# yusupov1alik/MPI-Jordan-crazy-acceleration

Measured on AMD Instinct MI355X. Metric: GFLOP/s + wall-clock, N=32768 dense Gauss-Jordan at 1/2/4/8 MI355X, higher is better.
Workload: dtype fp64

## Files before the change

### csrc/include/gj/device.hpp

```cpp
#pragma once

#include <cmath>
#include <limits>
#include <memory>
#include <string>

#include "gj/common.hpp"
#include "gj/layout.hpp"
#include "gj/pivot.hpp"

namespace gj {

enum class GenKind : int { AbsDiff = 0, Hilbert = 1, Identity = 2, Random = 3, Zero = 4, RandomShifted = 5 };

struct GenSpec {
  GenKind kind = GenKind::AbsDiff;
  uint64_t seed = 0;
};

enum class GemmOp : int { Acc = 0, Store = 1 };
enum class ALayout : int { RowMajor = 0, KMajor = 1 };

struct GemmExtra {
  static constexpr int kMaxZeroRows = 8;
  int64_t zc0 = 0, zc1 = 0;
  int nzr = 0;
  int64_t zr[kMaxZeroRows] = {};
  int64_t zh = 0;
  bool latency = false;
  bool lat_wide = false;
  bool lat_reg = false;
  void* tneg = nullptr;
  int64_t ldtneg = 0;
  int64_t tneg_cols = 0;
  int64_t skip_c0 = 0, skip_c1 = 0;
  const int32_t* owner_phys = nullptr;
  int64_t owner_p = 1, owner_k = 0;
  bool dense = false;
  int glds_build = 0;
  int glds_tile = 0;
  int c_nt = -1;
  const void* c_in = nullptr;
  int64_t ldc_in = 0;
  static constexpr int kRselWords = 8;
  uint64_t rsel[kRselWords] = {};
  int64_t rsel_m = 0;
  int64_t rsel_count() const {
    int64_t c = 0;
    for (int w = 0; w < kRselWords; ++w) c += __builtin_popcountll(rsel[w]);
    return c;
  }
  int64_t rsel_row(int64_t i) const {
    int64_t bl = i / rsel_m;
    const int64_t off = i - bl * rsel_m;
    for (int w = 0; w < kRselWords; ++w) {
      uint64_t x = rsel[w];
      const int c = __builtin_popcountll(x);
      if (bl < c) {
        for (; bl > 0; --bl) x &= x - 1;
        return (64 * w + __builtin_ctzll(x)) * rsel_m + off;
      }
// ... 215 lines not shown
```

### csrc/kernels/gemm.hip

```cpp
#include <hip/hip_runtime.h>

#include <stdexcept>

#include <cstdint>
#include <cstdlib>
#include <string>
#include <type_traits>
#include <utility>

#include "kernels.hpp"

namespace gj {
namespace kern {

constexpr int PADL = 16;
constexpr int kRecords = 0x7ffffff0;
constexpr int kOOB = 0x7ffffff8;

template <int BM_, int BN_, int BK_, int WM_, int WN_, int OCC_, int PF_ = 1>
struct Cfg {
  static constexpr int BM = BM_, BN = BN_, BK = BK_, WM = WM_, WN = WN_, OCC = OCC_;
  static constexpr int PF = PF_;
  static constexpr int NT = 64 * WM * WN;
  static constexpr int TM = BM / WM, TN = BN / WN;
// ... 89 lines not shown
struct GemmArgs {
  int64_t M, N, K;
  const void* A;
  int64_t lda;
  const void* B;
  int64_t ldb;
  void* C;
  int64_t ldc;
  int tiles_m, tiles_n;
  int64_t zc0, zc1;
  int64_t zr[GemmExtra::kMaxZeroRows];
  int64_t zh;
  int64_t n_real, blk_m, p, k;
  double* partial;
  int nparts;
  bool latency;
  bool lat_wide;
  bool lat_reg;
  bool c_overlap;
  int group;
  void* tneg;
  int64_t ldt, tncols;
  const int32_t* pred;
  int64_t pred_p, pred_k;
  bool dense;
  int build;
  int tile;
  uint64_t rsel[GemmExtra::kRselWords];
  int64_t rsel_m;
  int64_t skc0, skc1;
  const void* cin;
  int64_t ldcin;
  int c_nt;
};

__device__ __forceinline__ int64_t rsel_map(const GemmArgs& g, int64_t r) {
  int64_t bl = r / g.rsel_m;
  const int64_t off = r - bl * g.rsel_m;
#pragma unroll
  for (int w = 0; w < GemmExtra::kRselWords; ++w) {
    uint64_t x = g.rsel[w];
    const int c = __popcll(x);
    if (bl < c) {
      for (; bl > 0; --bl) x &= x - 1;
      return (64 * w + __ffsll((unsigned long long)x) - 1) * g.rsel_m + off;
    }
    bl -= c;
  }
  return 0;
}

__device__ __forceinline__ bool gemm_skipped(const GemmArgs& g) {
  if (g.pred == nullptr) return false;
  const int64_t gg = *g.pred;
  return gg < 0 || gg % g.pred_p != g.pred_k;
}

__device__ __forceinline__ int xcd_remap(int bid, int nwg) {
  const int q = nwg / 8, r = nwg % 8, x = bid % 8;
  return (x < r ? x * (q + 1) : r * (q + 1) + (x - r) * q) + bid / 8;
}

template <typename T, int AL, int MODE, typename CF>
__device__ __forceinline__ void gemm_tile(const GemmArgs& g, const int tile) {
  using MF = Mfma<T>;
  using acc_t = typename MF::acc_t;
// ... 307 lines not shown
  const int rlane = wm * TM + MF::rl(lane);
  const int clane = wn * TN + (lane & 15);
  const int Mt = (int)((g.M - m0L) < BM ? (g.M - m0L) : BM);
  const int Nt = (int)((g.N - n0) < BN ? (g.N - n0) : BN);
  const int64_t zlo = g.zc0 - n0, zhi = g.zc1 - n0;
  const int z0 = (int)(zlo < 0 ? 0 : (zlo > BN ? BN : zlo)), z1 = (int)(zhi < 0 ? 0 : (zhi > BN ? BN : zhi));
  int zr0[GemmExtra::kMaxZeroRows], zr1[GemmExtra::kMaxZeroRows];
#pragma unroll
  for (int z = 0; z < GemmExtra::kMaxZeroRows; ++z) {
    const int64_t lo = g.zr[z] - m0, hi = g.zr[z] + g.zh - m0;
    zr0[z] = (int)(lo < 0 ? 0 : (lo > BM ? BM : lo));
    zr1[z] = (int)(hi < 0 ? 0 : (hi > BM ? BM : hi));
  }
  __amdgpu_buffer_rsrc_t rc = rsrc(C + m0 * g.ldc + n0);
  const int cvoff = (rlane * ldc + clane) * ES;

  acc_t acc[MI][NJ];
  const int ldi = g.cin ? (int)g.ldcin : ldc;
  const __amdgpu_buffer_rsrc_t rci = g.cin ? rsrc(static_cast<const double*>(g.cin) + m0 * g.ldcin + n0) : rc;
  const int civoff = (rlane * ldi + clane) * ES;
  bool uni = Mt == BM && Nt == BN && g.cin == nullptr && g.rsel_m == 0;
  bool zin = MODE != MODE_ACC;
  if (MODE == MODE_ACC) {
    uni = uni && (z1 <= z0 || (z0 == 0 && z1 == BN));
    zin = z1 > z0;
#pragma unroll
    for (int z = 0; z < GemmExtra::kMaxZeroRows; ++z) {
      const int h = zr1[z] - zr0[z];
      uni = uni && (h <= 0 || h == BM);
      zin = zin || h > 0;
    }
  }
  if (g.tneg) uni = uni && (n0 >= g.tncols || n0 + BN <= g.tncols);
  auto load_c_masked = [&]() {
#pragma unroll
    for (int i = 0; i < MI; ++i)
#pragma unroll
      for (int q = 0; q < 4; ++q) {
        const int r = rlane + i * 16 + MF::rq(q);
        const int soff = (i * 16 + MF::rq(q)) * ldi * ES;
        bool zrow = false;
#pragma unroll
        for (int z = 0; z < GemmExtra::kMaxZeroRows; ++z) zrow |= (r >= zr0[z] && r < zr1[z]);
#pragma unroll
        for (int j = 0; j < NJ; ++j) {
          const int c = clane + j * 16;
          if (MODE == MODE_ACC) {
            const bool ok = r < Mt && c < Nt && !zrow && !(c >= z0 && c < z1);
            acc[i][j][q] = bload_c(rci, ok ? civoff + j * 16 * ES : kOOB, soff, g.c_nt & 1);
          } else {
            acc[i][j][q] = 0.0;
          }
        }
      }
  };
  auto load_c_uniform = [&](auto nt_c) {
#pragma unroll
    for (int i = 0; i < MI; ++i)
#pragma unroll
      for (int q = 0; q < 4; ++q) {
        const int soff = (i * 16 + MF::rq(q)) * ldc * ES;
#pragma unroll
        for (int j = 0; j < NJ; ++j) acc[i][j][q] = bload_c(rc, cvoff + j * 16 * ES, soff, decltype(nt_c)::value);
      }
  };
  auto load_c = [&]() {
    if (!uni) {
      load_c_masked();
    } else if (zin) {
#pragma unroll
      for (int i = 0; i < MI; ++i)
#pragma unroll
        for (int j = 0; j < NJ; ++j)
#pragma unroll
          for (int q = 0; q < 4; ++q) acc[i][j][q] = 0.0;
    } else if (g.c_nt & 1) {
      load_c_uniform(std::true_type{});
    } else {
      load_c_uniform(std::false_type{});
    }
  };
  if (!(MODE == MODE_ACC && g.c_overlap)) {
    load_c();
#pragma unroll
    for (int i = 0; i < MI; ++i)
#pragma unroll
      for (int j = 0; j < NJ; ++j)
#pragma unroll
        for (int q = 0; q < 4; ++q) asm volatile("" ::"v"(acc[i][j][q]));
  }

  const int acol = 2 * lane;
  const bool a_ok = (m0L + acol) < g.M;
  const int brow = BN == 128 ? wid : 2 * wid + (lane >> 5);
  const int bpos = BN == 128 ? 2 * lane : 2 * (lane & 31);
  const int bcol = bpos ^ ((brow & 1) * 16);
  const bool b_ok = (n0 + bcol) < g.N;
  auto brow_h = [&](int h) { return BN == 128 ? brow + 4 * h : brow + 8 * h; };
  auto blds_h = [&](int h) { return BN == 128 ? (wid + 4 * h) * BN : 2 * (wid + 4 * h) * BN; };
  __amdgpu_buffer_rsrc_t ra = rsrc(A + m0);
  __amdgpu_buffer_rsrc_t rb = rsrc(B + n0);
  const int Kd = (int)g.K;
  auto issue = [&](int kt) {
    double* st = lds + (kt % NS) * STAGE;
    const int k0 = kt * BK;
#pragma unroll
    for (int h = 0; h < BK / 4; ++h) {
      const int kr = wid + 4 * h;
      const bool ok = a_ok && (k0 + kr) < Kd;
      dma16(ra, st + kr * LDA, ok ? ((k0 + kr) * lda + acol) * ES : kOOB);
    }
#pragma unroll
    for (int h = 0; h < BPW; ++h) {
      const int br = brow_h(h);
      const bool okb = b_ok && (k0 + br) < Kd;
      dma16(rb, st + SA + blds_h(h), okb ? ((k0 + br) * ldb + bcol) * ES : kOOB);
    }
  };
  auto compute = [&](int kt) {
    const double* sa = lds + (kt % NS) * STAGE;
    const double* sb = sa + SA;
#pragma unroll
    for (int kk = 0; kk < BK; kk += 4) {
      double a[MI], b[NJ];
      const int kr = kk + (lane >> 4);
      const int sw = (kr & 1) * 16;
#pragma unroll
      for (int i = 0; i < MI; ++i) a[i] = sa[kr * LDA + wm * TM + i * 16 + (lane & 15)];
#pragma unroll
      for (int j = 0; j < NJ; ++j) b[j] = sb[kr * BN + ((wn * TN + j * 16 + (lane & 15)) ^ sw)];
#pragma unroll
      for (int i = 0; i < MI; ++i)
#pragma unroll
        for (int j = 0; j < NJ; ++j) acc[i][j] = MF::op(a[i], b[j], acc[i][j]);
    }
  };

  const int nk = (int)((g.K + BK - 1) / BK);
  const int pro = nk < NS - 1 ? nk : NS - 1;
  if constexpr (PEEL == 0) {
    for (int kt = 0; kt < pro; ++kt) issue(kt);
    if (MODE == MODE_ACC && g.c_overlap) {
      load_c();
      asm volatile("s_waitcnt vmcnt(0)" ::: "memory");
    } else {
      wait_pieces<PIECES>(pro - 1);
    }
    __builtin_amdgcn_s_barrier();
    for (int kt = 0; kt < nk; ++kt) {
      if (kt + NS - 1 < nk) issue(kt + NS - 1);
      compute(kt);
      const int last = (kt + NS - 1 < nk ? kt + NS - 1 : nk - 1);
      wait_pieces<PIECES>(last - (kt + 1) > 0 ? last - (kt + 1) : 0);
      asm volatile("s_waitcnt lgkmcnt(0)" ::: "memory");
      __builtin_amdgcn_s_barrier();
    }
  } else {
    const int nfull = Kd / BK;
    int va[BK / 4], vb[BPW];
#pragma unroll
    for (int h = 0; h < BK / 4; ++h) va[h] = a_ok ? ((wid + 4 * h) * lda + acol) * ES : kOOB;
#pragma unroll
    for (int h = 0; h < BPW; ++h) vb[h] = b_ok ? (brow_h(h) * ldb + bcol) * ES : kOOB;
    const int sa_step = __builtin_amdgcn_readfirstlane(BK * lda * ES);
    const int sb_step = __builtin_amdgcn_readfirstlane(BK * ldb * ES);
    for (int kt = 0; kt < pro; ++kt) issue(kt);
    if (MODE == MODE_ACC && g.c_overlap) {
      load_c();
      asm volatile("s_waitcnt vmcnt(0)" ::: "memory");
    } else {
      wait_pieces<PIECES>(pro - 1);
// ... 271 lines not shown
}
void set_glds_peel(int on) { g_glds_peel = on ? 1 : 0; }
static int g_glds_build = -1;
static int glds_build_forced() {
  if (g_glds_build < 0) {
    const char* e = getenv("GJ_GLDS_BUILD");
    const std::string v = e ? e : "";
    g_glds_build = v.empty() ? 0 : v == "2.5" ? 25 : v == "3.3" ? 33 : v == "2.3" ? 23 : v == "4.3" ? 43
                                                  : v == "16.2.3" ? 1623 : v == "3.2" ? 32 : -2;
    if (g_glds_build == -2) throw std::invalid_argument("GJ_GLDS_BUILD: 2.3 | 2.5 | 3.3 | 4.3 | 16.2.3 | 3.2");
  }
  return g_glds_build;
}
void set_glds_build(int b) {
  if (b != 0 && b != 23 && b != 25 && b != 33 && b != 43 && b != 1623 && b != 32)
    throw std::invalid_argument("glds build: 0 | 23 | 25 | 32 | 33 | 43 | 1623");
  g_glds_build = b;
}

static int g_glds_tile = -1;
static int glds_tile(const GemmArgs& a) {
  if (g_glds_tile < 0) {
    const char* e = getenv("GJ_GLDS_TILE");
    const int v = e ? std::atoi(e) : 0;
    if (v != 0 && v != 64 && v != 128) throw std::invalid_argument("GJ_GLDS_TILE: 64 | 128");
    g_glds_tile = v;
  }
  return g_glds_tile ? g_glds_tile : a.tile == 64 ? 64 : 128;
}
void set_glds_tile(int bn) {
  if (bn != 0 && bn != 64 && bn != 128) throw std::invalid_argument("glds tile: 0 (per launch) | 64 | 128");
  g_glds_tile = bn;
}

static int glds_cnt(int per_launch) {
  static const int forced = [] {
    const char* e = getenv("GJ_GLDS_CNT");
    return e ? (std::atoi(e) & 3) : -1;
  }();
  return forced >= 0 ? forced : per_launch > 0 ? (per_launch & 3) : 0;
}

static int glds_group() {
  static const int g = [] {
    const char* e = getenv("GJ_GLDS_GROUP");
    const int v = e ? std::atoi(e) : 4;
    return v > 0 ? v : 4;
  }();
  return g;
}

template <int MODE>
static void launch_glds(const GemmArgs& a0, hipStream_t s) {
  GemmArgs a = a0;
  const int forced0 = glds_build_forced();
  const int build0 = forced0 ? forced0 : a.build ? a.build : a.dense ? 25 : 23;
  if (glds_tile(a) == 128 && glds_peel() && build0 != 25) {
    a.tiles_m = (int)((a.M + glds::BM - 1) / glds::BM);
    a.tiles_n = (int)((a.N + 127) / 128);
    const int64_t nwg = (int64_t)a.tiles_m * a.tiles_n;
    if (nwg <= 0) return;
    a.group = glds_group();
    a.c_nt = glds_cnt(a.c_nt);
    g_last_gemm_kernel = build0 == 33 ? "glds64:t128:b33:peel" : build0 == 32 ? "glds64:t128:b32:peel" : "glds64:t128:b23:peel";
    if (build0 == 33)
      hipLaunchKernelGGL((gemm_glds_f64<MODE, 3, 3, 8, 1, 128>), dim3((unsigned)nwg), dim3(glds::NT), 0, s, a);
// ... 419 lines not shown
    case 9: return launch_cfg<T, AL, MODE, CfgBigPf>(a, s);
    default: return launch_cfg<T, AL, MODE, CfgBig>(a, s);
  }
}

static void fill_extra(GemmArgs& a, const GemmExtra* ex) {
  constexpr int64_t kNone = -(int64_t(1) << 62);
  a.zc0 = ex ? ex->zc0 : 0;
  a.zc1 = ex ? ex->zc1 : 0;
  a.zh = ex ? ex->zh : 0;
  for (int z = 0; z < GemmExtra::kMaxZeroRows; ++z) a.zr[z] = (ex && z < ex->nzr) ? ex->zr[z] : kNone;
  a.latency = ex ? ex->latency : false;
  a.lat_wide = ex ? ex->lat_wide : false;
  a.lat_reg = ex ? ex->lat_reg : false;
  a.c_overlap = glds_covl();
  a.tneg = ex ? ex->tneg : nullptr;
  a.ldt = ex ? ex->ldtneg : 0;
  a.tncols = (ex && ex->tneg_cols > 0) ? ex->tneg_cols : (int64_t(1) << 62);
  a.pred = ex ? ex->owner_phys : nullptr;
  a.pred_p = ex ? ex->owner_p : 1;
  a.pred_k = ex ? ex->owner_k : 0;
  a.dense = ex ? ex->dense : false;
  a.build = ex ? ex->glds_build : 0;
  a.tile = ex ? ex->glds_tile : 0;
  a.c_nt = ex ? ex->c_nt : -1;
  a.rsel_m = ex ? ex->rsel_m : 0;
  a.cin = ex ? ex->c_in : nullptr;
  a.skc0 = ex ? ex->skip_c0 : 0;
  a.skc1 = ex ? ex->skip_c1 : 0;
  if (a.skc1 > a.skc0 && (a.skc0 % 128 != 0 || a.skc1 % 128 != 0))
    throw Error(Status::BadArgs, "gemm: skip columns must be multiples of 128");
  a.ldcin = ex ? ex->ldc_in : 0;
  for (int w = 0; w < GemmExtra::kRselWords; ++w) a.rsel[w] = ex ? ex->rsel[w] : 0;
}

void gemm(DType dt, int op, int a_kmajor, int64_t M, int64_t N, int64_t K, const void* A,
          int64_t lda, const void* B, int64_t ldb, void* C, int64_t ldc, hipStream_t s,
          const GemmExtra* ex) {
  if (M <= 0 || N <= 0) return;
  GemmArgs a{};
  a.M = M; a.N = N; a.K = K; a.A = A; a.lda = lda; a.B = B; a.ldb = ldb; a.C = C; a.ldc = ldc;
  fill_extra(a, ex);
  if (a.tneg && a.ldt * 128 * (dt == DType::F64 ? 8 : 4) >= kRecords)
    throw Error(Status::BadArgs, "gemm: -C^T leading dimension too large for 32-bit buffer offsets");
  const int mode = op == 0 ? MODE_ACC : MODE_STORE;
#define GJ_DISPATCH(T)                                                        \
  if (a_kmajor) {                                                             \
    if (mode == MODE_ACC) launch<T, 1, MODE_ACC>(a, s);                       \
    else launch<T, 1, MODE_STORE>(a, s);                                      \
  } else {                                                                    \
    if (mode == MODE_ACC) launch<T, 0, MODE_ACC>(a, s);                       \
    else launch<T, 0, MODE_STORE>(a, s);                                      \
  }
  if (dt == DType::F64) {
    GJ_DISPATCH(double)
  } else {
    GJ_DISPATCH(float)
  }
#undef GJ_DISPATCH
}

void gemm_batch(DType dt, const GemmDesc* d, int n, hipStream_t s) {
  using CF = CfgSmall;
  static const bool lat_batch = !getenv("GJ_LAT_BATCH") || std::atoi(getenv("GJ_LAT_BATCH")) != 0;
  bool lat = lat_batch && dt == DType::F64 && n > 0;
  for (int e = 0; e < n && lat; ++e) {
// ... 74 lines not shown
```

### csrc/kernels/kernels.hpp

```cpp
#pragma once

#include <hip/hip_runtime.h>

#include "gj/common.hpp"
#include "gj/device.hpp"
#include "gj/layout.hpp"
#include "gj/pivot.hpp"

namespace gj {
namespace kern {

void gemm(DType dt, int op , int a_kmajor, int64_t M, int64_t N, int64_t K,
          const void* A, int64_t lda, const void* B, int64_t ldb, void* C, int64_t ldc,
          hipStream_t s, const GemmExtra* ex = nullptr);
void gemm_batch(DType dt, const GemmDesc* d, int n, hipStream_t s);
const char* last_gemm_kernel();
int residual_nparts(int64_t N);
int gemm_variant_id(const char* name);
void set_gemm_variant(int v);
void set_glds_peel(int on);
void set_glds_covl(int on);
void set_lat_glds(int on);
void set_lat_kernel(int mode);
void set_glds_build(int b);
void set_glds_tile(int bn);
void set_block_inverse_variant(int v);
int block_inverse_variant();
int block_inverse_variant_id(const char* name);
const char* block_inverse_kernel_name(DType dt, int64_t m, int variant);
void residual_partial(DType dt, int64_t M, int64_t N, int64_t K, const void* A, int64_t lda,
                      const void* B, int64_t ldb, int64_t n_real, int64_t blk_m, int64_t p,
                      int64_t k, double* partial, hipStream_t s);

void candidate_maxabs(DType dt, const void* Lt, int64_t ldl, double* scores, int32_t* valid,
                      const int32_t* used, const Layout& L, double thresh, hipStream_t s);
void gather_candidate(DType dt, void* sel, const void* Lt, int64_t ldl, const PivotRec* rec, const Layout& L,
                      hipStream_t s);
void commit_candidate(DType dt, void* inv_t, const void* inv1, const int32_t* valid1, const double* score1, double growth, PivotRec* rec,
                      const Layout& L, hipStream_t s);

void block_inverse(DType dt, const void* Lt, int64_t ldl, void* inv_t, double* scores,
                   int32_t* valid, const int32_t* used, const Layout& L, double thresh, int64_t nlive,
                   hipStream_t s, void* scratch, int* iscratch, int variant = -1);
bool block_inverse_mfma(DType dt, const void* Lt, int64_t ldl, void* inv_t, double* scores,
                        int32_t* valid, const int32_t* used, const Layout& L, double thresh, int64_t nlive,
                        hipStream_t s, const PivotSelectArgs* sel = nullptr);
bool block_inverse_select(DType dt, const void* Lt, int64_t ldl, void* inv_t, double* scores,
                          int32_t* valid, const int32_t* used, const Layout& L, double thresh, int64_t nlive,
                          hipStream_t s, const PivotSelectArgs& sel, int variant = -1, void* scratch = nullptr);
void set_block_inverse_probe(int32_t* piv_out);
int32_t* block_inverse_probe();
bool block_inverse_big(DType dt, const void* Lt, int64_t ldl, void* inv_t, double* scores, int32_t* valid,
                       const int32_t* used, const Layout& L, double thresh, int64_t nlive, hipStream_t s, void* scratch);
size_t block_inverse_big_scratch_bytes(DType dt, const Layout& L);
void block_inverse_huge(DType dt, const void* Lt, int64_t ldl, void* inv_t, double* scores, int32_t* valid,
                        const int32_t* used, const Layout& L, double thresh, int64_t nlive, hipStream_t s,
                        void* scratch);
bool block_inverse_co(DType dt, const void* Lt, int64_t ldl, void* inv_t, double* scores, int32_t* valid,
// ... 91 lines not shown
```

### csrc/python/module.cpp

```cpp
#include <pybind11/numpy.h>
#include <pybind11/pybind11.h>

#include <thread>
#include <pybind11/stl.h>

#include <hip/hip_runtime.h>

#include <cstring>
#include <memory>
#include <tuple>

#include "gj/async_host_device.hpp"
#include "gj/comms.hpp"
#include "gj/engine.hpp"
#include "gj/hip_device.hpp"
#include "gj/host_device.hpp"
#include "gj/io.hpp"
#include "gj/race_check.hpp"
#include "gj/runner.hpp"
#include "../kernels/kernels.hpp"

namespace py = pybind11;
using namespace gj;

// ... 181 lines not shown
      if (p) std::rethrow_exception(p);
    } catch (const Error& e) {
      py::object inst = gj_error(e.what());
      inst.attr("status") = (int)e.status();
      PyErr_SetObject(gj_error.ptr(), inst.ptr());
    }
  });

  mod.def("version", [] { return std::string("0.1.0"); });
  mod.def("device_count", [] {
    int n = 0;
    if (hipGetDeviceCount(&n) != hipSuccess) return 0;
    return n;
  });
  mod.def("rccl_unique_id", [] { return py::bytes(RcclComm::unique_id()); });
  mod.def("layout_real_rows",
          [](int64_t n, int64_t m, int64_t p, int64_t k) { return Layout::make(n, m, p, k).real_rows(); },
          "Layout::real_rows(): rank k's local rows whose global row is < n");
  mod.def("set_block_inverse_variant", [](const std::string& v) {
    kern::set_block_inverse_variant(kern::block_inverse_variant_id(v.c_str()));
  });
  mod.def("set_block_inverse_probe", [](uintptr_t p) { kern::set_block_inverse_probe(reinterpret_cast<int32_t*>(p)); },
          "test probe: device int32 buffer (nblk x m) receiving each candidate's pivot row per column; 0 = off");
  mod.def("set_gemm_variant", [](const std::string& v) { kern::set_gemm_variant(kern::gemm_variant_id(v.c_str())); });
  mod.def("set_glds_peel", [](bool on) { kern::set_glds_peel(on ? 1 : 0); },
          "fp64 LDS-DMA trailing-update kernel: the peeled, stage-unrolled main loop (GJ_GLDS_PEEL)");
  mod.def("set_glds_covl", [](bool on) { kern::set_glds_covl(on ? 1 : 0); },
          "fp64 LDS-DMA kernel: C loads overlapped with the first K slices (GJ_GLDS_COVL)");
  mod.def("set_glds_build", [](int b) { kern::set_glds_build(b); },
          "fp64 LDS-DMA trailing-update build for every launch: 23 | 25 | 33 | 43 | 1623, 0 = auto (GJ_GLDS_BUILD)");
  mod.def("set_glds_tile", [](int bn) { kern::set_glds_tile(bn); },
          "fp64 LDS-DMA trailing-update tile width for the 4-per-CU builds: 64 | 128 for every launch, 0 = per "
          "launch (the engine's choice; GJ_GLDS_TILE)");
  mod.def("set_lat_kernel", [](int mode) { kern::set_lat_kernel(mode); },
          "fp64 latency GEMMs on the register-fed small kernel: 1 / 0 for every launch, -1 per launch "
          "(GemmExtra::lat_reg; GJ_LAT_KERNEL)");
  mod.def("last_gemm_kernel", [] { return std::string(kern::last_gemm_kernel()); },
          "test probe: family / build name of the kernel this thread's last Device.gemm / gemm_batch ran "
          "('host' on the host executor)");
  mod.def("set_rhs_splitk", [](int s) { kern::set_rhs_splitk(s); },
          "test hook: K-split of the following Device.panel_rhs launches on the GPU (0 = auto, s >= 1 forces s)");
  mod.def("last_rhs_kernel", [] { return std::string(kern::last_rhs_kernel()); },
          "test probe: 'rhs<16|32|64>:<f64|f32>:<vec|scalar>:s<split>' of this thread's last Device.panel_rhs "
          "('host' on the host executor)");
  mod.def("set_rhs_t_split", [](int v) { kern::set_rhs_t_split(v); },
          "test hook: row split of the following Device.panel_rhs_t launches on the GPU (0 = auto, s >= 1 forces s)");
  mod.def("last_rhs_t_kernel", [] { return std::string(kern::last_rhs_t_kernel()); },
          "test probe: 'rhst<16|32|64>:<f64|f32>:<vec|scalar>:s<split>' of this thread's last Device.panel_rhs_t "
          "('host' on the host executor)");
  mod.def("last_abs_kernel", [] { return std::string(kern::last_abs_kernel()); },
          "test probe: 'abs<16|32|64>:<f64|f32>:<vec|scalar>:s<split>' of this thread's last Device.panel_abs_rhs, "
          "'abst...' of its last panel_abs_rhs_t ('host' on the host executors); the splits are those of "
          "set_rhs_splitk / set_rhs_t_split");
  mod.def("last_rank_update_kernel",[] { return std::string(kern::last_rank_update_kernel()); },
          "test probe: 'rku<k padded to 4>:<f64|f32>:<vec|scalar>' of this thread's last Device.rank_update "
          "('host' on the host executor)");
  mod.def("last_slogdet_kernel", [] { return std::string(kern::last_slogdet_kernel()); },
          "test probe: 'sld:<lds|glob>:<f64|f32>' of this thread's last Device.slogdet_batch ('host' on the "
          "host executor)");
  mod.def("last_equil_kernel", [] { return std::string(kern::last_equil_kernel()); },
          "test probe: 'eq:<rmax|cmax|scale>:<f64|f32>:<vec|scalar>' of this thread's last Device.abs_max_rows / "
          "abs_max_cols / scale_pow2 ('host' on the host executor)");
  mod.def("set_equil_col_split", [](int v) { kern::set_equil_col_split(v); },
          "test hook: row split of the following Device.abs_max_cols launches on the GPU (0 = auto, s >= 1 forces s)");
  mod.def("set_equil_nt", [](bool on) { kern::set_equil_nt(on ? 1 : 0); },
          "Device.scale_pow2 on the GPU: panel accesses with the non-temporal policy (default) or plain (measurements)");
  mod.def("set_lat_glds", [](bool on) { kern::set_lat_glds(on ? 1 : 0); },
          "every latency GEMM of >= 1024 rows on the LDS-DMA kernel (tests; the engine sets it per launch)");

  using U = uintptr_t;
  auto lay = [](int64_t n, int64_t m, int64_t p, int64_t k) { return Layout::make(n, m, p, k); };
  py::class_<Device, std::shared_ptr<Device>>(mod, "Device")
      .def_property_readonly("on_gpu", &Device::on_gpu)
      .def("describe", &Device::describe)
      .def("sync", &Device::sync_all, py::call_guard<py::gil_scoped_release>())
      .def("gemm",
           [](Device& d, const std::string& dt, const std::string& op, bool a_kmajor, int64_t M,
              int64_t N, int64_t K, U A, int64_t lda, U B, int64_t ldb, U C, int64_t ldc, int64_t zc0,
              int64_t zc1, std::vector<int64_t> zero_rows, int64_t zh, U tneg, int64_t ldtneg, bool latency,
              int64_t tneg_cols, bool dense, U c_in, int64_t ldc_in, std::vector<int64_t> row_blocks,
              int64_t row_block_m, int64_t skip_c0, int64_t skip_c1, py::object owner, bool lat_wide,
              bool lat_reg, int glds_build, int glds_tile, int c_nt) {
             GemmExtra ex;
             set_owner(ex, owner);
             ex.lat_wide = lat_wide;
             ex.lat_reg = lat_reg;
             ex.glds_build = glds_build;
             ex.glds_tile = glds_tile;
             ex.c_nt = c_nt;
             ex.dense = dense;
             ex.skip_c0 = skip_c0;
             ex.skip_c1 = skip_c1;
             ex.c_in = (const void*)c_in;
             ex.ldc_in = ldc_in;
             if (row_block_m > 0) {
               ex.rsel_m = row_block_m;
               for (int64_t b : row_blocks) {
                 if (b < 0 || b >= 64 * GemmExtra::kRselWords) throw std::invalid_argument("row block out of range");
                 ex.rsel[b / 64] |= uint64_t(1) << (b % 64);
               }
               if (M != ex.rsel_count() * row_block_m) throw std::invalid_argument("M != selected rows");
             }
             ex.tneg = (void*)tneg;
             ex.ldtneg = ldtneg;
             ex.tneg_cols = tneg_cols;
             ex.latency = latency;
             ex.zc0 = zc0;
             ex.zc1 = zc1;
             if (zero_rows.size() > (size_t)GemmExtra::kMaxZeroRows) throw std::invalid_argument("too many zero rows");
             ex.nzr = (int)zero_rows.size();
             for (size_t i = 0; i < zero_rows.size(); ++i) ex.zr[i] = zero_rows[i];
             ex.zh = zh;
             d.gemm(parse_dtype(dt), op == "store" ? GemmOp::Store : GemmOp::Acc,
                    a_kmajor ? ALayout::KMajor : ALayout::RowMajor, M, N, K, (const void*)A, lda,
                    (const void*)B, ldb, (void*)C, ldc, S_MAIN, ex);
             d.sync_stream(S_MAIN);
           },
           py::arg("dtype"), py::arg("op"), py::arg("a_kmajor"), py::arg("M"), py::arg("N"), py::arg("K"),
           py::arg("A"), py::arg("lda"), py::arg("B"), py::arg("ldb"), py::arg("C"), py::arg("ldc"),
           py::arg("zc0") = 0, py::arg("zc1") = 0, py::arg("zero_rows") = std::vector<int64_t>(),
           py::arg("zh") = 0, py::arg("tneg") = U(0), py::arg("ldtneg") = 0, py::arg("latency") = false,
           py::arg("tneg_cols") = 0, py::arg("dense") = false, py::arg("c_in") = U(0), py::arg("ldc_in") = 0,
           py::arg("row_blocks") = std::vector<int64_t>(), py::arg("row_block_m") = 0, py::arg("skip_c0") = 0,
           py::arg("skip_c1") = 0, py::arg("owner") = py::none(), py::arg("lat_wide") = false,
           py::arg("lat_reg") = false, py::arg("glds_build") = 0, py::arg("glds_tile") = 0, py::arg("c_nt") = -1)
      .def("gemm_batch",
           [](Device& d, const std::string& dt, const std::vector<py::tuple>& ps) {
             std::vector<GemmDesc> v(ps.size());
             for (size_t i = 0; i < ps.size(); ++i) {
               const py::tuple& t = ps[i];
               if (t.size() < 10 || t.size() > 12) throw std::invalid_argument("gemm_batch: 10 to 12 fields per product");
               GemmDesc& g = v[i];
               g.op = t[0].cast<std::string>() == "store" ? GemmOp::Store : GemmOp::Acc;
               g.M = t[1].cast<int64_t>(); g.N = t[2].cast<int64_t>(); g.K = t[3].cast<int64_t>();
               g.A = (const void*)t[4].cast<U>(); g.lda = t[5].cast<int64_t>();
               g.B = (const void*)t[6].cast<U>(); g.ldb = t[7].cast<int64_t>();
               g.C = (void*)t[8].cast<U>(); g.ldc = t[9].cast<int64_t>();
               if (t.size() > 10) g.ex.lat_reg = t[10].cast<bool>();
               if (t.size() > 11) set_owner(g.ex, t[11]);
             }
             d.gemm_batch(parse_dtype(dt), v.data(), (int)v.size(), S_MAIN);
             d.sync_stream(S_MAIN);
           },
           py::arg("dtype"), py::arg("products"))
      .def("generate",
           [lay](Device& d, const std::string& dt, U X, int64_t n, int64_t m, int64_t p, int64_t k,
                 const std::string& kind, uint64_t seed) {
             GenSpec g;
             g.kind = parse_gen(kind);
             g.seed = seed;
             d.generate(parse_dtype(dt), (void*)X, lay(n, m, p, k), g, S_MAIN);
             d.sync_stream(S_MAIN);
           })
      .def("extract_neg_t",
           [](Device& d, const std::string& dt, U Lt, int64_t ldl, U X, int64_t ldx, int64_t rows,
              int64_t col0, int64_t m) {
             d.extract_neg_t(parse_dtype(dt), (void*)Lt, ldl, (const void*)X, ldx, rows, col0, m, S_MAIN);
             d.sync_stream(S_MAIN);
// ... 1120 lines not shown
```

### csrc/runtime/host_device.cpp

```cpp
#include <chrono>
#include "gj/host_device.hpp"

#include <algorithm>
#include <atomic>
#include <type_traits>
#include <cmath>
#include <cstdlib>
#include <cstring>
#include <limits>
#include <thread>
#include <vector>

#include "gj/gen.hpp"

namespace gj {

namespace {

template <typename F>
void parallel_for(int64_t n, int nthreads, F f) {
  if (n <= 0) return;
  int nt = (int)std::min<int64_t>(nthreads, n);
  if (nt <= 1) {
    for (int64_t i = 0; i < n; ++i) f(i);
    return;
  }
  std::vector<std::thread> th;
  th.reserve(nt);
  for (int w = 0; w < nt; ++w)
    th.emplace_back([=, &f] {
      for (int64_t i = w; i < n; i += nt) f(i);
    });
  for (auto& t : th) t.join();
}

template <typename T>
T* tp(void* p) {
  return static_cast<T*>(p);
}
template <typename T>
const T* tp(const void* p) {
  return static_cast<const T*>(p);
}

template <typename T>
void gemm_t(GemmOp op, ALayout al, int64_t M, int64_t N, int64_t K, const T* A, int64_t lda,
            const T* B, int64_t ldb, T* C, int64_t ldc, int nthreads, const GemmExtra& ex) {
  if (ex.owner_phys) {
    const int64_t g = *ex.owner_phys;
    if (g < 0 || g % ex.owner_p != ex.owner_k) return;
  }
  parallel_for(M, nthreads, [&](int64_t il) {
    const int64_t i = ex.rsel_m > 0 ? ex.rsel_row(il) : il;
    bool zrow = false;
    for (int z = 0; z < ex.nzr; ++z) zrow |= (i >= ex.zr[z] && i < ex.zr[z] + ex.zh);
    std::vector<double> acc(N, 0.0);
    for (int64_t k = 0; k < K; ++k) {
      const double a = (al == ALayout::RowMajor) ? (double)A[i * lda + k] : (double)A[k * lda + i];
      const T* b = B + k * ldb;
      for (int64_t j = 0; j < N; ++j)
        if (!(j >= ex.skip_c0 && j < ex.skip_c1)) acc[j] += a * (double)b[j];
    }
    T* c = C + i * ldc;
    const T* ci = ex.c_in ? static_cast<const T*>(ex.c_in) + i * ex.ldc_in : c;
    const auto skip = [&](int64_t j) { return j >= ex.skip_c0 && j < ex.skip_c1; };
    if (op == GemmOp::Acc) {
      for (int64_t j = 0; j < N; ++j)
        if (!skip(j)) c[j] = (T)((zrow || (j >= ex.zc0 && j < ex.zc1) ? 0.0 : (double)ci[j]) + acc[j]);
    } else {
      for (int64_t j = 0; j < N; ++j)
        if (!skip(j)) c[j] = (T)acc[j];
    }
    if (ex.tneg) {
      const int64_t nt = ex.tneg_cols > 0 ? std::min(ex.tneg_cols, N) : N;
      for (int64_t j = 0; j < nt; ++j)
        if (!skip(j)) static_cast<T*>(ex.tneg)[j * ex.ldtneg + i] = -c[j];
    }
  });
}

inline bool sweep_inverse(std::vector<double>& W, int64_t m, double thresh, std::vector<int64_t>& prow,
                          double limit) {
  std::vector<char> used(m, 0);
  for (int64_t k = 0; k < m; ++k) {
// ... 752 lines not shown
```

### csrc/solver/engine.cpp

```cpp
#include "gj/engine.hpp"

#include "gj/io.hpp"
#include "../kernels/kernels.hpp"

#include <rocprofiler-sdk-roctx/roctx.h>

#include <algorithm>
#include <atomic>
#include <chrono>
#include <cmath>
#include <cstdio>
#include <cstdlib>
#include <cstring>
#include <limits>

#include <unistd.h>
#include <thread>

namespace gj {

namespace {
double now_s() {
  using clk = std::chrono::steady_clock;
  return std::chrono::duration<double>(clk::now().time_since_epoch()).count();
// ... 548 lines not shown
        dev_.pivot_select_single(scores_, valid_, L_, (int32_t)t, pos_, phys_at_, used_, seq_, myrec_,
                                 piv_dev_, &piv_host_[par], S_SIDE);
      prof_end(PH_PIVOT, pe, S_SIDE);
      dbg_sync();
      return;
    }
    if (!fused) dev_.pivot_local(scores_, valid_, used_, pos_, L_, myrec_, S_SIDE);
    prof_end(PH_PIVOT, pe, S_SIDE);
  }
  if (hang_step_ == t) {
    dev_.host_access(&piv_host_[par].step, sizeof(int32_t), true);
    piv_host_[par].step = -1;
    return;
  }
  pe = prof_begin(S_SIDE);
  comm_.set_step(t);
  if (L_.p > 1) comm_.allgather(dev_, myrec_, recs_, sizeof(PivotRec), S_SIDE);
  count_comm(SolveStats::CK_RECORDS, double(sizeof(PivotRec)) * L_.p);
  dev_.host_access(&piv_host_[par].step, sizeof(int32_t), true);
  piv_host_[par].step = -1;
  dev_.pivot_global(L_.p > 1 ? recs_ : myrec_, (int32_t)L_.p, (int32_t)t, pos_, phys_at_, used_, seq_, piv_dev_,
                    &piv_host_[par], S_SIDE);
  if (vparts_ && L_.p > 1)
    vhash(panel_of(t), vslot(V_RECS, t - panel_t0(panel_of(t))), recs_, (int64_t)sizeof(PivotRec) * L_.p, (int64_t)sizeof(PivotRec) * L_.p,
          1, S_SIDE);
  prof_end(PH_EXCHANGE, pe, S_SIDE);
  dbg_sync();
}

GemmExtra Engine::pivot_rows_extra(int par, int64_t nsteps) const {
  GemmExtra ex;
  ex.zh = L_.m;
  for (int64_t j = 0; j < nsteps; ++j)
    if (piv_[par][j].owner == L_.k) ex.zr[ex.nzr++] = (piv_[par][j].phys / L_.p) * L_.m;
  return ex;
}

void Engine::begin_panel(int64_t v) {
  cur_step_ = panel_t0(v);
  cur_phase_ = "pivot search";
  dev_.wait(S_SIDE, ev_L_);
  if (v >= 2 && !dropped("cp")) dev_.wait(S_SIDE, ev_cp_[v & 1]);
  select(panel_t0(v), At_[v % 3]);
}

bool Engine::factor_panel(int64_t v, SolveStats& st, double& host_wait) {
  const int par = (int)(v & 1);
  const int64_t m = L_.m, rows = L_.rows, npad = L_.npad, dm = (int64_t)d_ * m;
  const int64_t t0 = panel_t0(v), q = panel_q(v);
  const size_t es = esz();
  const bool ahead = host_free_chain();
  for (int64_t j = 0; j < q; ++j) {
    const int64_t t = t0 + j;
    cur_step_ = t;
    cur_phase_ = "pivot search";
    void* Lt = elem(At_[v % 3], j * m * rows);
    if (j > 0) {
      if (step_events_) dev_.wait(S_SIDE, ev_pp_[par][j - 1]);
      if (vparts_)
        vhash(v, vslot(V_PP, j - 1), elem(PP_[par], (j - 1) * m * dm), dm * (int64_t)es, dm * (int64_t)es, m,
              S_SIDE);
      const int pe = prof_begin(S_SIDE);
      if (rows > 0) {
        GemmExtra ex = chain_sel_[par];
        ex.latency = true;
        ex.lat_wide = lat_wide_;
        ex.lat_reg = lat_reg_;
// ... 414 lines not shown
    int64_t ra[2], rb[2], nr = 0;
    int64_t sk0 = 0, sk1 = 0;
    if (has_next && x0 >= c0 && x0 < c1) {
      const int64_t al = dev_.skip_align();
      if ((x0 - c0) % al == 0 && (x1 - c0) % al == 0 && x1 <= c1 && skip_cols_) {
        ra[0] = c0; rb[0] = c1; nr = 1;
        sk0 = x0 - c0;
        sk1 = x1 - c0;
      } else {
        if (x0 > c0) { ra[nr] = c0; rb[nr] = x0; ++nr; }
        if (c1 > x1) { ra[nr] = x1; rb[nr] = c1; ++nr; }
      }
    } else {
      ra[0] = c0; rb[0] = c1; nr = 1;
    }
    const int pieces = (main_split_ == 2 || (main_split_ == 1 && i == 0)) ? 2 : 1;
    const int64_t s_abs0 = c0 + sk0, s_abs1 = c0 + sk1;
    if (rows > 0)
      for (int64_t z = 0; z < nr; ++z) {
        int64_t cut[3] = {ra[z], rb[z], rb[z]};
        int np = 1;
        if (pieces == 2 && rb[z] - ra[z] >= 256) {
          cut[1] = ra[z] + ((rb[z] - ra[z]) / 256) * 128;
          np = 2;
        }
        for (int h = 0; h < np; ++h) {
          const int64_t a = cut[h], b = cut[h + 1];
          GemmExtra ex = prows;
          const int64_t s0 = std::max(s_abs0, a), s1 = std::min(s_abs1, b);
          ex.skip_c0 = s1 > s0 ? s0 - a : 0;
          ex.skip_c1 = s1 > s0 ? s1 - a : 0;
          ex.zc0 = pc0 - a;
          ex.zc1 = pc1 - a;
          ex.dense = dense_gemm_;
          ex.c_nt = main_cnt_;
          dev_.gemm(opt_.dtype, GemmOp::Acc, ALayout::KMajor, rows, b - a, K, At, rows,
                    rb_chunk(par, c) + (a - c0) * (int64_t)esz(), W, elem(X_, a), npad, ms, ex);
        }
      }
    prof_end(PH_UPDATE, pe, ms);
    if (i + 1 == C && vlocal_on()) vlocal_hash(u, V_LE, true, ms);
    dev_.record(ev_c_[c], ms);
  }
  dbg_sync();
}

SolveStats Engine::solve() {
  try {
    return solve_steps();
  } catch (const Error& e) {
    if (e.status() != Status::CommError) throw;
    throw Error(Status::CommError, "rank " + std::to_string(L_.k) + "/" + std::to_string(L_.p) + ", step " +
                                       std::to_string(cur_step_) + " of " + std::to_string(L_.Nr) +
                                       ", phase " + cur_phase_ + ": " + e.what());
  }
}

SolveStats Engine::solve_steps() {
  GJ_REQUIRE(!solved_, "solve(): input panel already consumed; load the matrix again");
  det_ready_ = det_cached_ = false;
  cur_step_ = -1;
  cur_phase_ = "norm";
  SolveStats st;
  const int64_t m = L_.m, Nr = L_.Nr, rows = L_.rows, npad = L_.npad;
  pmarks_.clear();
  pev_next_ = 0;
// ... 588 lines not shown
```

### mpi_jordan_crazy_acceleration_amd/ops/__init__.py

```python
from __future__ import annotations

import functools

import torch

from .._native import load_native

_DT = {torch.float64: "fp64", torch.float32: "fp32"}


@functools.lru_cache(maxsize=None)
def _hip(idx: int):
    return load_native().hip_device(idx)


@functools.lru_cache(maxsize=None)
def _host():
    return load_native().host_device(0)


def device_for(t: torch.Tensor):
    if t.is_cuda:
        torch.cuda.synchronize(t.device)
        return _hip(t.device.index if t.device.index is not None else torch.cuda.current_device())
    return _host()


def _p(t: torch.Tensor) -> int:
    return t.data_ptr()


def gemm(A: torch.Tensor, B: torch.Tensor, C: torch.Tensor, op: str = "acc", a_kmajor: bool = False,
         zero_cols=(0, 0), zero_rows=(), zero_row_height: int = 0, tneg: torch.Tensor = None,
         latency: bool = False, dense: bool = False, c_in: torch.Tensor = None, row_blocks=None,
         row_block_m: int = 0, skip_cols=(0, 0), owner=None, lat_wide: bool = False, lat_reg: bool = False,
         glds_build: int = 0, glds_tile: int = 0, c_nt: int = -1) -> torch.Tensor:
    assert A.dtype == B.dtype == C.dtype and A.stride(-1) == 1 and B.stride(-1) == 1 and C.stride(-1) == 1
    M, N = C.shape
    K = A.shape[0] if a_kmajor else A.shape[1]
    tp, ldt, tcols = 0, 0, 0
    if tneg is not None:
        assert tneg.dtype == C.dtype and tneg.shape[1] == M and 0 < tneg.shape[0] <= N and tneg.stride(-1) == 1
        tp, ldt, tcols = _p(tneg), tneg.stride(0), tneg.shape[0]
    cp, ldci = 0, 0
    if c_in is not None:
        assert c_in.dtype == C.dtype and c_in.shape == C.shape and c_in.stride(-1) == 1
        cp, ldci = _p(c_in), c_in.stride(0)
    rb = [int(b) for b in (row_blocks or [])]
    Msel = len(rb) * int(row_block_m) if row_block_m else M
    device_for(C).gemm(_DT[C.dtype], op, a_kmajor, Msel, N, K, _p(A), A.stride(0), _p(B), B.stride(0), _p(C),
                       C.stride(0), int(zero_cols[0]), int(zero_cols[1]), [int(r) for r in zero_rows],
                       int(zero_row_height), tp, ldt, bool(latency), tcols, bool(dense), cp, ldci, rb,
                       int(row_block_m), int(skip_cols[0]), int(skip_cols[1]), owner=_owner(owner, C),
                       lat_wide=bool(lat_wide), lat_reg=bool(lat_reg), glds_build=int(glds_build),
                       glds_tile=int(glds_tile), c_nt=int(c_nt))
    return C


def _owner(owner, C):
    if owner is None:
        return None
    phys, p, k = owner
    if phys is not None:
        assert phys.dtype == torch.int32 and phys.device == C.device and phys.numel() >= 1
    return (None if phys is None else _p(phys), int(p), int(k))


def gemm_batch(products) -> None:
    if not products:
        return
    C0 = products[0][3]
    descs = []
    for item in products:
        op, At, B, C = item[:4]
        extra = item[4] if len(item) > 4 else {}
        assert At.dtype == B.dtype == C.dtype == C0.dtype and At.stride(-1) == 1 and B.stride(-1) == 1
        assert C.stride(-1) == 1
        M, N = C.shape
        descs.append((op, M, N, At.shape[0], _p(At), At.stride(0), _p(B), B.stride(0), _p(C), C.stride(0),
                      bool(extra.get("lat_reg", False)), _owner(extra.get("owner"), C)))
    device_for(C0).gemm_batch(_DT[C0.dtype], descs)


def generate(X: torch.Tensor, n: int, m: int, p: int = 1, k: int = 0, kind: str = "absdiff", seed: int = 0) -> torch.Tensor:
    device_for(X).generate(_DT[X.dtype], _p(X), n, m, p, k, kind, seed)
    return X


# ... 231 lines not shown
```

Measured before the change: 69140.

## Skip known-zero K ranges in trailing-update GEMM tiles

Adds per-launch promises (zero-row k0 offsets and a zero-column k step) that let each uniform GEMM tile start its K loop past a prefix where the A rows or B columns are structurally zero in the blocked Gauss-Jordan update. The engine fills these promises from the pivot-step structure, and the kernel shifts the A/B buffer bases and shortens nk accordingly. This is meant to remove wasted fp64 MFMA work on the triangular zero portions. The host reference path checks the promises, and the feature is gated off when drop-wait mode is active.

```diff
diff --git a/csrc/include/gj/device.hpp b/csrc/include/gj/device.hpp
--- a/csrc/include/gj/device.hpp
+++ b/csrc/include/gj/device.hpp
@@ -27,6 +27,8 @@
   int nzr = 0;
   int64_t zr[kMaxZeroRows] = {};
   int64_t zh = 0;
+  int64_t zr_k0[kMaxZeroRows] = {};
+  int64_t zc_kstep = 0;
   bool latency = false;
   bool lat_wide = false;
   bool lat_reg = false;
diff --git a/csrc/kernels/gemm.hip b/csrc/kernels/gemm.hip
--- a/csrc/kernels/gemm.hip
+++ b/csrc/kernels/gemm.hip
@@ -145,6 +145,8 @@
   const void* cin;
   int64_t ldcin;
   int c_nt;
+  int zr_k0[GemmExtra::kMaxZeroRows];
+  int zc_kstep;
 };
 
 __device__ __forceinline__ int64_t rsel_map(const GemmArgs& g, int64_t r) {
@@ -518,6 +520,19 @@
     }
   }
   if (g.tneg) uni = uni && (n0 >= g.tncols || n0 + BN <= g.tncols);
+  int kbeg = 0;
+  if (MODE == MODE_ACC && uni && zin) {
+    int kr = -1;
+#pragma unroll
+    for (int z = 0; z < GemmExtra::kMaxZeroRows; ++z)
+      if (zr1[z] - zr0[z] == BM) kr = (kr < 0 || g.zr_k0[z] < kr) ? g.zr_k0[z] : kr;
+    if (kr < 0) kr = 0;
+    int kc = 0;
+    if (z1 > z0 && g.zc_kstep > 0) kc = ((int)(n0 - g.zc0) / g.zc_kstep) * g.zc_kstep;
+    kbeg = kr > kc ? kr : kc;
+    kbeg = kbeg < (int)g.K ? kbeg : (int)g.K;
+    kbeg -= kbeg % BK;
+  }
   auto load_c_masked = [&]() {
 #pragma unroll
     for (int i = 0; i < MI; ++i)
@@ -584,9 +599,9 @@
   const bool b_ok = (n0 + bcol) < g.N;
   auto brow_h = [&](int h) { return BN == 128 ? brow + 4 * h : brow + 8 * h; };
   auto blds_h = [&](int h) { return BN == 128 ? (wid + 4 * h) * BN : 2 * (wid + 4 * h) * BN; };
-  __amdgpu_buffer_rsrc_t ra = rsrc(A + m0);
-  __amdgpu_buffer_rsrc_t rb = rsrc(B + n0);
-  const int Kd = (int)g.K;
+  __amdgpu_buffer_rsrc_t ra = rsrc(A + m0 + (int64_t)kbeg * g.lda);
+  __amdgpu_buffer_rsrc_t rb = rsrc(B + n0 + (int64_t)kbeg * g.ldb);
+  const int Kd = (int)g.K - kbeg;
   auto issue = [&](int kt) {
     double* st = lds + (kt % NS) * STAGE;
     const int k0 = kt * BK;
@@ -622,7 +637,7 @@
     }
   };
 
-  const int nk = (int)((g.K + BK - 1) / BK);
+  const int nk = (Kd + BK - 1) / BK;
   const int pro = nk < NS - 1 ? nk : NS - 1;
   if constexpr (PEEL == 0) {
     for (int kt = 0; kt < pro; ++kt) issue(kt);
@@ -960,6 +975,9 @@
   if (bn != 0 && bn != 64 && bn != 128) throw std::invalid_argument("glds tile: 0 (per launch) | 64 | 128");
   g_glds_tile = bn;
 }
+
+static bool g_gemm_kskip = true;
+void set_gemm_kskip(bool on) { g_gemm_kskip = on; }
 
 static int glds_cnt(int per_launch) {
   static const int forced = [] {
@@ -1445,6 +1463,9 @@
     throw Error(Status::BadArgs, "gemm: skip columns must be multiples of 128");
   a.ldcin = ex ? ex->ldc_in : 0;
   for (int w = 0; w < GemmExtra::kRselWords; ++w) a.rsel[w] = ex ? ex->rsel[w] : 0;
+  const auto k32 = [&](int64_t k) { return (int)std::min<int64_t>(std::max<int64_t>(k, 0), std::min<int64_t>(a.K, INT32_MAX)); };
+  for (int z = 0; z < GemmExtra::kMaxZeroRows; ++z) a.zr_k0[z] = (ex && g_gemm_kskip && z < ex->nzr) ? k32(ex->zr_k0[z]) : 0;
+  a.zc_kstep = (ex && g_gemm_kskip && ex->zc_kstep > 0 && ex->zc_kstep <= INT32_MAX) ? (int)ex->zc_kstep : 0;
 }
 
 void gemm(DType dt, int op, int a_kmajor, int64_t M, int64_t N, int64_t K, const void* A,
diff --git a/csrc/kernels/kernels.hpp b/csrc/kernels/kernels.hpp
--- a/csrc/kernels/kernels.hpp
+++ b/csrc/kernels/kernels.hpp
@@ -24,6 +24,7 @@
 void set_lat_kernel(int mode);
 void set_glds_build(int b);
 void set_glds_tile(int bn);
+void set_gemm_kskip(bool on);
 void set_block_inverse_variant(int v);
 int block_inverse_variant();
 int block_inverse_variant_id(const char* name);
diff --git a/csrc/python/module.cpp b/csrc/python/module.cpp
--- a/csrc/python/module.cpp
+++ b/csrc/python/module.cpp
@@ -237,6 +237,9 @@
   mod.def("set_glds_tile", [](int bn) { kern::set_glds_tile(bn); },
           "fp64 LDS-DMA trailing-update tile width for the 4-per-CU builds: 64 | 128 for every launch, 0 = per "
           "launch (the engine's choice; GJ_GLDS_TILE)");
+  mod.def("set_gemm_kskip", [](bool on) { kern::set_gemm_kskip(on); },
+          "GPU GEMM kernels: act on the zero-operand promises GemmExtra::zr_k0 / zc_kstep (default) or run the "
+          "full K (tests and A/B runs; the results are bit-identical)");
   mod.def("set_lat_kernel", [](int mode) { kern::set_lat_kernel(mode); },
           "fp64 latency GEMMs on the register-fed small kernel: 1 / 0 for every launch, -1 per launch "
           "(GemmExtra::lat_reg; GJ_LAT_KERNEL)");
@@ -285,7 +288,8 @@
               int64_t zc1, std::vector<int64_t> zero_rows, int64_t zh, U tneg, int64_t ldtneg, bool latency,
               int64_t tneg_cols, bool dense, U c_in, int64_t ldc_in, std::vector<int64_t> row_blocks,
               int64_t row_block_m, int64_t skip_c0, int64_t skip_c1, py::object owner, bool lat_wide,
-              bool lat_reg, int glds_build, int glds_tile, int c_nt) {
+              bool lat_reg, int glds_build, int glds_tile, int c_nt, std::vector<int64_t> zr_k0,
+              int64_t zc_kstep) {
              GemmExtra ex;
              set_owner(ex, owner);
              ex.lat_wide = lat_wide;
@@ -316,6 +320,9 @@
              ex.nzr = (int)zero_rows.size();
              for (size_t i = 0; i < zero_rows.size(); ++i) ex.zr[i] = zero_rows[i];
              ex.zh = zh;
+             if (!zr_k0.empty() && zr_k0.size() != zero_rows.size()) throw std::invalid_argument("zr_k0: one per zero row");
+             for (size_t i = 0; i < zr_k0.size(); ++i) ex.zr_k0[i] = zr_k0[i];
+             ex.zc_kstep = zc_kstep;
              d.gemm(parse_dtype(dt), op == "store" ? GemmOp::Store : GemmOp::Acc,
                     a_kmajor ? ALayout::KMajor : ALayout::RowMajor, M, N, K, (const void*)A, lda,
                     (const void*)B, ldb, (void*)C, ldc, S_MAIN, ex);
@@ -328,7 +335,8 @@
            py::arg("tneg_cols") = 0, py::arg("dense") = false, py::arg("c_in") = U(0), py::arg("ldc_in") = 0,
            py::arg("row_blocks") = std::vector<int64_t>(), py::arg("row_block_m") = 0, py::arg("skip_c0") = 0,
            py::arg("skip_c1") = 0, py::arg("owner") = py::none(), py::arg("lat_wide") = false,
-           py::arg("lat_reg") = false, py::arg("glds_build") = 0, py::arg("glds_tile") = 0, py::arg("c_nt") = -1)
+           py::arg("lat_reg") = false, py::arg("glds_build") = 0, py::arg("glds_tile") = 0, py::arg("c_nt") = -1,
+           py::arg("zr_k0") = std::vector<int64_t>(), py::arg("zc_kstep") = 0)
       .def("gemm_batch",
            [](Device& d, const std::string& dt, const std::vector<py::tuple>& ps) {
              std::vector<GemmDesc> v(ps.size());
diff --git a/csrc/runtime/host_device.cpp b/csrc/runtime/host_device.cpp
--- a/csrc/runtime/host_device.cpp
+++ b/csrc/runtime/host_device.cpp
@@ -44,12 +44,40 @@
 }
 
 template <typename T>
+void check_zero_promise(ALayout al, int64_t M, int64_t N, int64_t K, const T* A, int64_t lda, const T* B,
+                        int64_t ldb, const GemmExtra& ex) {
+  const auto fail = [&](const char* what, int64_t k, int64_t i) {
+    throw Error(Status::BadArgs, "gemm " + std::to_string(M) + " x " + std::to_string(N) + " x " + std::to_string(K) +
+                                     ": promised-zero element of " + what + " is not zero at k = " + std::to_string(k) +
+                                     ", " + (what[0] == 'A' ? "row " : "column ") + std::to_string(i));
+  };
+  for (int z = 0; z < ex.nzr; ++z) {
+    const int64_t kz = std::min(ex.zr_k0[z], K);
+    if (kz <= 0) continue;
+    for (int64_t il = 0; il < M; ++il) {
+      const int64_t i = ex.rsel_m > 0 ? ex.rsel_row(il) : il;
+      if (i < ex.zr[z] || i >= ex.zr[z] + ex.zh) continue;
+      for (int64_t k = 0; k < kz; ++k)
+        if ((al == ALayout::RowMajor ? A[i * lda + k] : A[k * lda + i]) != T(0)) fail("A (GemmExtra::zr_k0)", k, i);
+    }
+  }
+  if (ex.zc_kstep > 0)
+    for (int64_t x = std::max<int64_t>(ex.zc0, 0); x < std::min(ex.zc1, N); ++x) {
+      if (x >= ex.skip_c0 && x < ex.skip_c1) continue;
+      const int64_t kx = std::min(((x - ex.zc0) / ex.zc_kstep) * ex.zc_kstep, K);
+      for (int64_t k = 0; k < kx; ++k)
+        if (B[k * ldb + x] != T(0)) fail("B (GemmExtra::zc_kstep)", k, x);
+    }
+}
+
+template <typename T>
 void gemm_t(GemmOp op, ALayout al, int64_t M, int64_t N, int64_t K, const T* A, int64_t lda,
             const T* B, int64_t ldb, T* C, int64_t ldc, int nthreads, const GemmExtra& ex) {
   if (ex.owner_phys) {
     const int64_t g = *ex.owner_phys;
     if (g < 0 || g % ex.owner_p != ex.owner_k) return;
   }
+  if (op == GemmOp::Acc) check_zero_promise(al, M, N, K, A, lda, B, ldb, ex);
   parallel_for(M, nthreads, [&](int64_t il) {
     const int64_t i = ex.rsel_m > 0 ? ex.rsel_row(il) : il;
     bool zrow = false;
diff --git a/csrc/solver/engine.cpp b/csrc/solver/engine.cpp
--- a/csrc/solver/engine.cpp
+++ b/csrc/solver/engine.cpp
@@ -604,7 +604,10 @@
   GemmExtra ex;
   ex.zh = L_.m;
   for (int64_t j = 0; j < nsteps; ++j)
-    if (piv_[par][j].owner == L_.k) ex.zr[ex.nzr++] = (piv_[par][j].phys / L_.p) * L_.m;
+    if (piv_[par][j].owner == L_.k) {
+      ex.zr_k0[ex.nzr] = drop_wait_.empty() ? j * L_.m : 0;
+      ex.zr[ex.nzr++] = (piv_[par][j].phys / L_.p) * L_.m;
+    }
   return ex;
 }
 
@@ -1085,6 +1088,7 @@
           ex.skip_c1 = s1 > s0 ? s1 - a : 0;
           ex.zc0 = pc0 - a;
           ex.zc1 = pc1 - a;
+          ex.zc_kstep = drop_wait_.empty() ? m : 0;
           ex.dense = dense_gemm_;
           ex.c_nt = main_cnt_;
           dev_.gemm(opt_.dtype, GemmOp::Acc, ALayout::KMajor, rows, b - a, K, At, rows,
diff --git a/mpi_jordan_crazy_acceleration_amd/ops/__init__.py b/mpi_jordan_crazy_acceleration_amd/ops/__init__.py
--- a/mpi_jordan_crazy_acceleration_amd/ops/__init__.py
+++ b/mpi_jordan_crazy_acceleration_amd/ops/__init__.py
@@ -34,7 +34,8 @@
          zero_cols=(0, 0), zero_rows=(), zero_row_height: int = 0, tneg: torch.Tensor = None,
          latency: bool = False, dense: bool = False, c_in: torch.Tensor = None, row_blocks=None,
          row_block_m: int = 0, skip_cols=(0, 0), owner=None, lat_wide: bool = False, lat_reg: bool = False,
-         glds_build: int = 0, glds_tile: int = 0, c_nt: int = -1) -> torch.Tensor:
+         glds_build: int = 0, glds_tile: int = 0, c_nt: int = -1, zero_row_k0=(),
+         zero_col_kstep: int = 0) -> torch.Tensor:
     assert A.dtype == B.dtype == C.dtype and A.stride(-1) == 1 and B.stride(-1) == 1 and C.stride(-1) == 1
     M, N = C.shape
     K = A.shape[0] if a_kmajor else A.shape[1]
@@ -53,7 +54,8 @@
                        int(zero_row_height), tp, ldt, bool(latency), tcols, bool(dense), cp, ldci, rb,
                        int(row_block_m), int(skip_cols[0]), int(skip_cols[1]), owner=_owner(owner, C),
                        lat_wide=bool(lat_wide), lat_reg=bool(lat_reg), glds_build=int(glds_build),
-                       glds_tile=int(glds_tile), c_nt=int(c_nt))
+                       glds_tile=int(glds_tile), c_nt=int(c_nt), zr_k0=[int(k) for k in zero_row_k0],
+                       zc_kstep=int(zero_col_kstep))
     return C
 
 
```

Measured after the change: 69440 (median of 6 runs). No clear change (+0.4%).
